# UMich-CURLY/SE3ET

Measured on AMD Instinct MI355X. Metric: point-cloud pairs/sec (fwd), SE3ET-E 5k-pt pairs, higher is better.
Workload: dtype f32

## Files before the change

### include/se3et_hip.h

```cpp
#ifndef SE3ET_HIP_H_
#define SE3ET_HIP_H_

#include <stddef.h>
#include <stdint.h>

#ifdef __cplusplus
extern "C" {
#endif

#define SE3_OK 0
#define SE3_ERR_INVALID_ARG 1
#define SE3_ERR_UNSUPPORTED 2
#define SE3_ERR_LAUNCH 3
#define SE3_ERR_WORKSPACE 4

#define SE3_MAX_BATCH 32
#define SE3_MAX_NEIGHBOR_LIMIT 64

const char* se3_version(void);
const char* se3_last_error(void);
void se3_debug_set_sinkhorn_variant(int variant);
unsigned long long se3_debug_dense_saturated_rows(int reset);
unsigned long long se3_debug_attention_saturated(int reset);
void se3_debug_kernel_timing(int enable);
int se3_debug_kernel_timing_collect_ex(float* microseconds, int* tags, double* aux, int capacity);

int se3_radius_neighbors(const float* q_points, int64_t nq, const float* s_points, int64_t ns,
                         const int64_t* q_lengths_host, const int64_t* s_lengths_host, int batch, float radius,
                         int limit, int64_t* neighbors, int32_t* max_count, void* stream);

int se3_neighbor_table_trim(const int64_t* full, int64_t rows, int full_width, int width, const int64_t* pair_row_ends_host,
                            const int* pair_widths_host, int num_pairs, int64_t* out, void* stream);
size_t se3_radius_grid_workspace_bytes(int64_t ns, int batch);
int se3_radius_grid_build(const float* s_points, int64_t ns, const int64_t* s_lengths_host, int batch, float radius,
                          void* workspace, size_t workspace_bytes, void* stream);
int se3_radius_neighbors_grid(const float* q_points, int64_t nq, const int64_t* q_lengths_host, const int64_t* s_lengths_host,
                              int64_t ns, int batch, const void* grid_workspace, float radius, int limit, int64_t* neighbors,
                              int32_t* max_count, int max_count_is_zero, void* stream);

int se3_radius_count_hist(const float* q_points, int64_t nq, const float* s_points, int64_t ns, const int64_t* q_lengths_host,
                          const int64_t* s_lengths_host, int batch, float radius, const void* grid_workspace, int hist_n,
                          const int* slot_of_cloud_host, int num_slots, int32_t* hist, int32_t* dropped, int32_t* max_count, void* stream);

int se3_radius_neighbors_ties(const float* q_points, int64_t nq, const float* s_points, int64_t ns, const int64_t* q_lengths_host,
                              const int64_t* s_lengths_host, int batch, float radius, int limit, int64_t* neighbors, int32_t* max_count,
                              int32_t* tie_rows, int32_t* tie_count, void* stream);
int se3_radius_neighbors_grid_ties(const float* q_points, int64_t nq, const int64_t* q_lengths_host, const int64_t* s_lengths_host,
                                   int64_t ns, int batch, const void* grid_workspace, float radius, int limit, int64_t* neighbors,
                                   int32_t* max_count, int max_count_is_zero, int32_t* tie_rows, int32_t* tie_count, void* stream);
size_t se3_kdtree_max_bytes(int64_t ns, int batch);
int se3_kdtree_build_host(const float* s_points_host, int64_t ns, const int64_t* s_lengths_host, int batch, void* tree_host, size_t capacity,
                          size_t* used_bytes);
size_t se3_radius_tie_scratch_bytes(int64_t num_tie_rows, int max_hits);
int se3_radius_neighbors_tie_order(const float* q_points, int64_t nq, const float* s_points, int64_t ns, const int64_t* q_lengths_host,
                                   const int64_t* s_lengths_host, int batch, const void* tree_dev, float radius, int limit,
                                   const int32_t* tie_rows, int64_t num_tie_rows, int max_hits, void* scratch, size_t scratch_bytes,
                                   int64_t* neighbors, void* stream);
int se3_debug_radius_tie_order_host(const float* q_points, int64_t nq, const float* s_points, int64_t ns, const int64_t* q_lengths,
                                    const int64_t* s_lengths, int batch, const void* tree_host, float radius, int limit,
                                    const int32_t* tie_rows, int64_t num_tie_rows, int max_hits, int64_t* neighbors, int* overflowed);
int64_t se3_debug_std_sort_host(const unsigned long long* keys, int64_t n, int mode);

size_t se3_grid_subsample_workspace_bytes(int64_t n, int batch);
int se3_grid_subsample(const float* points, const float* normals, int64_t n, const int64_t* lengths_host, int batch,
                       float voxel_size, float* s_points, float* s_normals, int64_t* s_lengths, void* workspace,
                       size_t workspace_bytes, void* stream);
int se3_grid_subsample_dev(const float* points, const float* normals, int64_t n_rows, const int64_t* lengths_dev, int batch,
                           float voxel_size, float* s_points, float* s_normals, int64_t* s_lengths, void* workspace,
                           size_t workspace_bytes, void* stream);

int se3_log_sinkhorn_fwd(const float* scores, const uint8_t* row_masks, const uint8_t* col_masks, const float* alpha,
                         int batch, int rows, int cols, int iterations, float inf, float* out, void* stream);
int se3_log_sinkhorn_bwd(const float* scores, const uint8_t* row_masks, const uint8_t* col_masks, const float* alpha,
                         const float* grad_out, int batch, int rows, int cols, int iterations, float inf, float* grad_scores,
                         float* grad_alpha_partial, void* stream);

size_t se3_group_norm_workspace_bytes(int64_t rows, int channels, int groups);
int se3_group_norm_fwd(const float* x, const float* x_bias, const float* residual, const float* weight, const float* bias,
                       int64_t rows, int channels, int groups, float eps, int apply_leaky_relu, float slope, float* out,
                       void* workspace, size_t workspace_bytes, void* stream);

int se3_group_norm_segments_fwd(const float* x, const float* x_bias, const float* residual, const float* weight,
                                const float* bias, int64_t rows, int channels, int groups,
                                const int64_t* segment_row_offsets_host, int num_segments, float eps, int apply_leaky_relu,
                                float slope, float* out, void* workspace, size_t workspace_bytes, void* stream);
size_t se3_group_norm_bwd_workspace_bytes(int channels);
int se3_group_norm_segments_bwd(const float* x, const float* x_bias, const float* residual, const float* weight, const float* bias,
                                const float* grad_out, int64_t rows, int channels, int groups, const int64_t* segment_row_offsets_host,
                                int num_segments, float eps, int apply_leaky_relu, float slope, float* grad_x, float* grad_residual,
                                float* grad_params, void* workspace, size_t workspace_bytes, void* stream);

size_t se3_group_norm_stats_workspace_bytes(int channels);
int se3_group_norm_stats(const float* x, const float* in_affine, float in_slope, const float* x_bias, const float* weight, const float* bias,
                         int64_t rows, int channels, int groups, const int64_t* segment_row_offsets_host, int num_segments, float eps,
                         float* affine_out, void* workspace, size_t workspace_bytes, void* stream);
int se3_group_norm_apply(const float* x, const float* affine_a, float slope_a, const float* affine_b, float slope_b, const float* residual,
                         const float* residual_affine, float final_slope, int64_t rows, int channels,
                         const int64_t* segment_row_offsets_host, int num_segments, int blocked_layout, float* out, void* stream);
int se3_group_norm_apply_amax(const float* x, const float* affine_a, float slope_a, const float* affine_b, float slope_b, const float* residual,
                              const float* residual_affine, float final_slope, int64_t rows, int channels,
                              const int64_t* segment_row_offsets_host, int num_segments, int blocked_layout, float* out, float* amax_out,
                              void* stream);
size_t se3_dense_norm_workspace_bytes(int groups);
int se3_dense_norm_fwd(const float* x, int64_t rows, int in_features, const float* in_affine_a, float in_slope_a, const float* in_affine_b,
                       float in_slope_b, const void* weight_pieces, int out_features, const float* linear_bias, const float* norm_weight,
                       const float* norm_bias, int groups, float eps, const int64_t* segment_row_offsets_host, int num_segments, float* out,
                       float* affine_out, void* workspace, size_t workspace_bytes, void* stream);
int se3_dense_residual_fwd(const float* x, int64_t rows, int in_features, const float* in_affine_a, float in_slope_a, const float* in_affine_b,
                           float in_slope_b, const void* weight_pieces, const float* affine, const float* x2, int in_features2,
                           const void* weight_pieces2, const float* affine2, const float* residual, int out_features, float final_slope,
                           const int64_t* segment_row_offsets_host, int num_segments, float* out, void* stream);
int se3_linear_stream(const float* x, int64_t rows, int in_features, int64_t x_row_stride, const void* weight_pieces, const float* bias,
                      int out_features, int apply_relu, float* out, int64_t out_row_stride, void* stream);
int se3_linear_stream_transposed(const float* x, int64_t rows, int in_features, int64_t x_row_stride, const void* weight_pieces,
                                 const float* bias, int out_features, int block_rows, float* out_t, int64_t ld, void* stream);

int se3_add_layer_norm_fwd(const float* hidden, const float* hidden_bias, const float* residual, const float* weight,
                           const float* bias, int64_t rows, int64_t residual_rows, int channels, float eps, float* out,
                           void* stream);
int se3_add_layer_norm_bwd(const float* hidden, const float* hidden_bias, const float* residual, const float* weight,
                           const float* grad_out, int64_t rows, int64_t residual_rows, int channels, float eps, float* grad_hidden,
                           float* grad_params, void* stream);

size_t se3_linear_weight_pieces_bytes(int out_features, int in_features);
int se3_linear_split_weights_f16(const float* weight, int out_features, int in_features, void* pieces, void* stream);
int se3_linear_f16(const float* x, int64_t rows, int in_features, int64_t x_row_stride, const void* weight_pieces, const float* bias,
                   int out_features, int apply_relu, float* out, int64_t out_row_stride, void* stream);

int se3_gather_rows_padded(const float* x, const int64_t* idx, int64_t n, int64_t m, int64_t width, float* out,
                           void* stream);
int se3_neighbor_max_pool(const float* x, const int64_t* idx, int64_t n, int64_t m, int nn, int64_t width, float* out,
                          void* stream);
int se3_neighbor_max_pool_bwd(const float* x, const int64_t* idx, const float* dout, int64_t n, int64_t m, int nn, int64_t width,
                              float* dx, void* stream);
int se3_anchor_max(const float* x, int num_anchors, int64_t rows, int channels, int64_t anchor_stride, int64_t row_stride,
// ... 774 lines not shown
```

### se3et_amd/csrc/radius_ties.hip

```cpp
#define SE3_EXACT_FP 1
#include "common.h"
#include "kdtree_ref.h"
#include <string.h>
#include <memory>
#include <thread>

namespace {

struct KdCloud {
  int32_t node_base;
  int32_t perm_base;
  int32_t n_nodes, n_points;
  float lo[3], hi[3];
  int32_t pad[2];
};
struct KdNode {
  int32_t kid0, kid1;
  int32_t first, last;
  int32_t axis;
  float low_end, high_start;
  int32_t pad;
};
struct KdHeader {
  int32_t magic, batch;
  int64_t total_nodes, total_points;
  int64_t off_clouds, off_perm, off_nodes;
  int64_t pad[2];
};
constexpr int32_t kMagic = 0x6b645433;
static_assert(sizeof(KdCloud) == 48 && sizeof(KdNode) == 32 && sizeof(KdHeader) == 64, "flattened k-d tree layout");

struct Batch {
  int64_t q_start[SE3_MAX_BATCH], q_count[SE3_MAX_BATCH], s_start[SE3_MAX_BATCH], s_count[SE3_MAX_BATCH];
  int n;
};

struct Strip {
  unsigned long long* base;
  int64_t stride;
  __host__ __device__ __forceinline__ unsigned long long get(int k) const { return base[(int64_t)k * stride]; }
  __host__ __device__ __forceinline__ void set(int k, unsigned long long v) const { base[(int64_t)k * stride] = v; }
};
__host__ __device__ __forceinline__ bool less_d2(unsigned long long a, unsigned long long b) { return (unsigned)(a >> 32) < (unsigned)(b >> 32); }

__host__ __device__ void adjust_heap(const Strip& s, int first, int hole, int len, unsigned long long value) {
  const int top = hole;
  int child = hole;
  while (child < (len - 1) / 2) {
    child = 2 * (child + 1);
    if (less_d2(s.get(first + child), s.get(first + child - 1))) child--;
    s.set(first + hole, s.get(first + child));
    hole = child;
  }
  if ((len & 1) == 0 && child == (len - 2) / 2) {
    child = 2 * (child + 1);
    s.set(first + hole, s.get(first + child - 1));
    hole = child - 1;
  }
  int parent = (hole - 1) / 2;
  while (hole > top && less_d2(s.get(first + parent), value)) {
    s.set(first + hole, s.get(first + parent));
    hole = parent;
    parent = (hole - 1) / 2;
  }
  s.set(first + hole, value);
}
__host__ __device__ void heap_sort(const Strip& s, int first, int last) {
  const int len = last - first;
  if (len >= 2) {
    for (int parent = (len - 2) / 2;; parent--) {
      adjust_heap(s, first, parent, len, s.get(first + parent));
      if (parent == 0) break;
    }
  }
  for (int end = last; end - first > 1;) {
    --end;
    const unsigned long long value = s.get(end);
    s.set(end, s.get(first));
    adjust_heap(s, first, 0, end - first, value);
  }
}
__host__ __device__ __forceinline__ void swap_at(const Strip& s, int a, int b) {
  const unsigned long long x = s.get(a), y = s.get(b);
  s.set(a, y);
  s.set(b, x);
}
__host__ __device__ __forceinline__ void linear_insert(const Strip& s, int last) {
  const unsigned long long val = s.get(last);
  int next = last - 1;
  while (less_d2(val, s.get(next))) {
    s.set(last, s.get(next));
    last = next;
    --next;
  }
  s.set(last, val);
}
__host__ __device__ void insertion_sort(const Strip& s, int first, int last) {
  if (first == last) return;
  for (int i = first + 1; i != last; ++i) {
    if (less_d2(s.get(i), s.get(first))) {
      const unsigned long long val = s.get(i);
      for (int k = i; k > first; k--) s.set(k, s.get(k - 1));
      s.set(first, val);
    } else {
      linear_insert(s, i);
    }
  }
}
struct Stacks {
  int* i;
  float* a;
  float* b;
  int stride;
};
constexpr int kMaxDepth = 48;

__host__ __device__ void std_sort(const Strip& s, int n, const Stacks& K) {
  if (n <= 0) return;
  constexpr int kThreshold = 16;
  int depth0 = 0;
  while ((2 << depth0) <= n) depth0++;
  int sp = 1;
  K.i[0] = 0 | (n << 16);
  K.a[0] = __builtin_bit_cast(float, 2 * depth0);
  while (sp > 0) {
    --sp;
    const int packed = K.i[sp * K.stride];
    int first = packed & 0xffff, last = (int)((unsigned)packed >> 16), depth = __builtin_bit_cast(int, K.a[sp * K.stride]);
    while (last - first > kThreshold) {
      if (depth == 0) {
        heap_sort(s, first, last);
        break;
      }
      --depth;
      const int mid = first + (last - first) / 2, a = first + 1, b = mid, c = last - 1;
      const unsigned long long va = s.get(a), vb = s.get(b), vc = s.get(c);
      int med;
      if (less_d2(va, vb)) med = less_d2(vb, vc) ? b : (less_d2(va, vc) ? c : a);
      else med = less_d2(va, vc) ? a : (less_d2(vb, vc) ? c : b);
      swap_at(s, first, med);
      const unsigned long long pivot = s.get(first);
      int lo = first + 1, hi = last;
      for (;;) {
        while (less_d2(s.get(lo), pivot)) ++lo;
        --hi;
        while (less_d2(pivot, s.get(hi))) --hi;
        if (!(lo < hi)) break;
        swap_at(s, lo, hi);
        ++lo;
      }
      if (sp < kMaxDepth) {
        K.i[sp * K.stride] = lo | (last << 16);
        K.a[sp * K.stride] = __builtin_bit_cast(float, depth);
        sp++;
      }
      last = lo;
    }
  }
  if (n > kThreshold) {
    insertion_sort(s, 0, kThreshold);
    for (int i = kThreshold; i < n; ++i) linear_insert(s, i);
  } else {
    insertion_sort(s, 0, n);
  }
}


__host__ __device__ bool tie_row(const float* __restrict__ q, const float* __restrict__ s, const Batch& bt, const unsigned char* __restrict__ tree,
                                 float r2, int limit, int64_t row, int max_hits, const Strip& strip, const Stacks& K, int64_t ns_total,
                                 int64_t* __restrict__ out) {
  int b = 0;
  while (b + 1 < bt.n && row >= bt.q_start[b] + bt.q_count[b]) b++;
  const KdHeader* H = reinterpret_cast<const KdHeader*>(tree);
  const KdCloud cl = reinterpret_cast<const KdCloud*>(tree + H->off_clouds)[b];
  const int32_t* perm = reinterpret_cast<const int32_t*>(tree + H->off_perm) + cl.perm_base;
  const KdNode* nodes = reinterpret_cast<const KdNode*>(tree + H->off_nodes) + cl.node_base;
  const float* sp = s + 3 * bt.s_start[b];
  const float qv[3] = {q[3 * row], q[3 * row + 1], q[3 * row + 2]};
  int n = 0;
  bool over = false;
  if (cl.n_points > 0) {
    float side[3] = {0.f, 0.f, 0.f}, outside = 0.f;
    for (int d = 0; d < 3; d++) {
      if (qv[d] < cl.lo[d]) { side[d] = (qv[d] - cl.lo[d]) * (qv[d] - cl.lo[d]); outside += side[d]; }
      if (qv[d] > cl.hi[d]) { side[d] = (qv[d] - cl.hi[d]) * (qv[d] - cl.hi[d]); outside += side[d]; }
    }
    int sp_ = 1;
    K.i[0] = 0;
    K.a[0] = outside;
    while (sp_ > 0) {
      const int top = (sp_ - 1) * K.stride;
      const int word = K.i[top], node = word & 0x3fffffff, stage = (int)((unsigned)word >> 30);
      const float f_outside = K.a[top];
      const KdNode nd = nodes[node];
      if (nd.kid0 < 0) {
        for (int k = nd.first; k < nd.last; k++) {
          const int j = perm[k];
          const float dx = qv[0] - sp[3 * j], dy = qv[1] - sp[3 * j + 1], dz = qv[2] - sp[3 * j + 2];
          float d2 = dx * dx;
          d2 += dy * dy;
          d2 += dz * dz;
          if (d2 < r2) {
            if (n < max_hits) strip.set(n, ((unsigned long long)__builtin_bit_cast(unsigned, d2) << 32) | (unsigned)(bt.s_start[b] + j));
            else over = true;
            n += n < max_hits ? 1 : 0;
          }
        }
        sp_--;
        continue;
      }
      const float v = nd.axis == 0 ? qv[0] : (nd.axis == 1 ? qv[1] : qv[2]);
      const float to_low = v - nd.low_end, to_high = v - nd.high_start;
      const bool low_first = (to_low + to_high) < 0;
      const float gap = low_first ? to_high * to_high : to_low * to_low;
      if (stage == 0) {
        K.i[top] = node | (1 << 30);
        if (sp_ < kMaxDepth) { K.i[sp_ * K.stride] = low_first ? nd.kid0 : nd.kid1; K.a[sp_ * K.stride] = f_outside; sp_++; } else { over = true; sp_--; }
      } else if (stage == 1) {
        const float kept = nd.axis == 0 ? side[0] : (nd.axis == 1 ? side[1] : side[2]);
        const float far_outside = f_outside + gap - kept;
        if (far_outside * 1.0f <= r2) {
          K.b[top] = kept;
          K.i[top] = node | (2 << 30);
          if (nd.axis == 0) side[0] = gap; else if (nd.axis == 1) side[1] = gap; else side[2] = gap;
          if (sp_ < kMaxDepth) { K.i[sp_ * K.stride] = low_first ? nd.kid1 : nd.kid0; K.a[sp_ * K.stride] = far_outside; sp_++; } else { over = true; sp_--; }
        } else {
          sp_--;
        }
      } else {
        const float kept = K.b[top];
        if (nd.axis == 0) side[0] = kept; else if (nd.axis == 1) side[1] = kept; else side[2] = kept;
        sp_--;
      }
    }
  }
  if (n >= 65536) over = true;
  if (over) return false;
  std_sort(strip, n, K);
  for (int k = 0; k < limit; k++) out[row * limit + k] = k < n ? (int64_t)(unsigned)(strip.get(k) & 0xffffffffull) : ns_total;
  return true;
}

__global__ __launch_bounds__(64) void radius_tie_rows_kernel(const float* __restrict__ q, const float* __restrict__ s, Batch bt,
                                                             const unsigned char* __restrict__ tree, float r2, int limit,
                                                             const int32_t* __restrict__ rows, int64_t num_rows, int max_hits,
                                                             unsigned long long* __restrict__ scratch, int64_t ns_total,
                                                             int64_t* __restrict__ out, int32_t* __restrict__ overflow) {
  __shared__ int stk_i[kMaxDepth * 64];
  __shared__ float stk_a[kMaxDepth * 64], stk_b[kMaxDepth * 64];
  const int64_t r = (int64_t)blockIdx.x * blockDim.x + threadIdx.x;
  if (r >= num_rows) return;
  const Stacks K{stk_i + threadIdx.x, stk_a + threadIdx.x, stk_b + threadIdx.x, 64};
  if (!tie_row(q, s, bt, tree, r2, limit, rows[r], max_hits, Strip{scratch + r, num_rows}, K, ns_total, out)) atomicAdd(overflow, 1);
}

int fill_batch(Batch* bt, const int64_t* q_len, const int64_t* s_len, int batch, int64_t nq, int64_t ns) {
  int64_t qs = 0, ss = 0;
  bt->n = batch;
  for (int b = 0; b < batch; b++) {
    if (q_len[b] < 0 || s_len[b] < 0) return 1;
    bt->q_start[b] = qs; bt->q_count[b] = q_len[b];
    bt->s_start[b] = ss; bt->s_count[b] = s_len[b];
    qs += q_len[b]; ss += s_len[b];
  }
  return qs != nq || ss != ns;
}

}

extern "C" size_t se3_kdtree_max_bytes(int64_t ns, int batch) {
  if (ns < 0 || batch < 1 || batch > SE3_MAX_BATCH) return 0;
  return se3_align256(sizeof(KdHeader)) + se3_align256(sizeof(KdCloud) * (size_t)batch) + se3_align256(sizeof(int32_t) * (size_t)(ns + 1)) +
         se3_align256(sizeof(KdNode) * (size_t)(2 * ns + batch));
}

extern "C" int se3_kdtree_build_host(const float* s_points_host, int64_t ns, const int64_t* s_lengths_host, int batch, void* tree_host,
                                     size_t capacity, size_t* used_bytes) {
  SE3_REQUIRE(s_points_host && s_lengths_host && tree_host && used_bytes, SE3_ERR_INVALID_ARG, "kdtree_build_host: null pointer");
  SE3_REQUIRE(batch >= 1 && batch <= SE3_MAX_BATCH && ns >= 0 && ns < (1ll << 30), SE3_ERR_INVALID_ARG, "kdtree_build_host: bad batch / size");
  SE3_REQUIRE(capacity >= se3_kdtree_max_bytes(ns, batch), SE3_ERR_WORKSPACE, "kdtree_build_host: buffer too small");
  unsigned char* base = (unsigned char*)tree_host;
  KdHeader H{};
  H.magic = kMagic;
  H.batch = batch;
  H.off_clouds = (int64_t)se3_align256(sizeof(KdHeader));
  H.off_perm = H.off_clouds + (int64_t)se3_align256(sizeof(KdCloud) * (size_t)batch);
  H.off_nodes = H.off_perm + (int64_t)se3_align256(sizeof(int32_t) * (size_t)(ns + 1));
  KdCloud* clouds = (KdCloud*)(base + H.off_clouds);
  int32_t* perm = (int32_t*)(base + H.off_perm);
  KdNode* nodes = (KdNode*)(base + H.off_nodes);
  std::vector<int64_t> start((size_t)batch + 1, 0);
  for (int b = 0; b < batch; b++) {
    SE3_REQUIRE(s_lengths_host[b] >= 0 && start[(size_t)b] + s_lengths_host[b] <= ns, SE3_ERR_INVALID_ARG, "kdtree_build_host: lengths exceed the point count");
    start[(size_t)b + 1] = start[(size_t)b] + s_lengths_host[b];
  }
  std::vector<std::unique_ptr<se3_kd::KdTree>> trees((size_t)batch);
  auto build_one = [&](int b) {
    const int64_t n = s_lengths_host[b];
    if (n > 0) trees[(size_t)b].reset(new se3_kd::KdTree(s_points_host + 3 * start[(size_t)b], n));
  };
  if (batch > 1 && ns >= 4096) {
    for (int b0 = 0; b0 < batch; b0 += 16) {
      std::vector<std::thread> pool;
      for (int b = b0; b < batch && b < b0 + 16; b++) pool.emplace_back(build_one, b);
      for (auto& t : pool) t.join();
    }
  } else {
    for (int b = 0; b < batch; b++) build_one(b);
  }
  int64_t s0 = 0, n0 = 0;
  for (int b = 0; b < batch; b++) {
    const int64_t n = s_lengths_host[b];
    KdCloud c{};
    c.node_base = (int32_t)n0;
    c.perm_base = (int32_t)s0;
    c.n_points = (int32_t)n;
    if (n > 0) {
      const se3_kd::KdTree& tree = *trees[(size_t)b];
      const auto& tn = tree.nodes();
      const auto& tp = tree.perm();
      c.n_nodes = (int32_t)tn.size();
      for (int d = 0; d < 3; d++) { c.lo[d] = tree.box_lo()[d]; c.hi[d] = tree.box_hi()[d]; }
      for (size_t k = 0; k < tp.size(); k++) perm[s0 + (int64_t)k] = (int32_t)tp[k];
      for (size_t k = 0; k < tn.size(); k++) {
        KdNode o{};
        o.kid0 = tn[k].kid[0]; o.kid1 = tn[k].kid[1];
        o.first = (int32_t)tn[k].first; o.last = (int32_t)tn[k].last;
        o.axis = tn[k].axis; o.low_end = tn[k].low_end; o.high_start = tn[k].high_start;
        nodes[n0 + (int64_t)k] = o;
      }
    }
    clouds[b] = c;
    s0 += n;
    n0 += c.n_nodes;
  }
  SE3_REQUIRE(s0 == ns, SE3_ERR_INVALID_ARG, "kdtree_build_host: lengths do not sum to ns");
  H.total_nodes = n0;
  H.total_points = ns;
  memcpy(base, &H, sizeof(H));
  *used_bytes = (size_t)H.off_nodes + sizeof(KdNode) * (size_t)n0;
  return SE3_OK;
}

extern "C" size_t se3_radius_tie_scratch_bytes(int64_t num_rows, int max_hits) {
  if (num_rows < 0 || max_hits < 0) return 0;
  return se3_align256(sizeof(unsigned long long) * (size_t)num_rows * (size_t)(max_hits > 0 ? max_hits : 1)) + 256;
}

extern "C" int se3_radius_neighbors_tie_order(const float* q_points, int64_t nq, const float* s_points, int64_t ns, const int64_t* q_lengths_host,
                                              const int64_t* s_lengths_host, int batch, const void* tree_dev, float radius, int limit,
                                              const int32_t* tie_rows, int64_t num_tie_rows, int max_hits, void* scratch, size_t scratch_bytes,
                                              int64_t* neighbors, void* stream) {
  SE3_REQUIRE(q_points && s_points && q_lengths_host && s_lengths_host && tree_dev && tie_rows && scratch && neighbors, SE3_ERR_INVALID_ARG,
              "radius_neighbors_tie_order: null pointer");
  SE3_REQUIRE(batch >= 1 && batch <= SE3_MAX_BATCH && limit >= 1 && limit <= SE3_MAX_NEIGHBOR_LIMIT && max_hits >= 1, SE3_ERR_INVALID_ARG,
              "radius_neighbors_tie_order: bad batch / limit / max_hits");
  SE3_REQUIRE(scratch_bytes >= se3_radius_tie_scratch_bytes(num_tie_rows, max_hits), SE3_ERR_WORKSPACE, "radius_neighbors_tie_order: scratch too small");
  Batch bt;
  SE3_REQUIRE(fill_batch(&bt, q_lengths_host, s_lengths_host, batch, nq, ns) == 0, SE3_ERR_INVALID_ARG,
              "radius_neighbors_tie_order: lengths do not sum to the sizes");
  if (num_tie_rows <= 0) return SE3_OK;
  hipStream_t st = (hipStream_t)stream;
  int32_t* overflow = (int32_t*)((char*)scratch + se3_radius_tie_scratch_bytes(num_tie_rows, max_hits) - 256);
  if (hipMemsetAsync(overflow, 0, sizeof(int32_t), st) != hipSuccess) {
    se3_set_error("radius_neighbors_tie_order: memset failed");
    return SE3_ERR_LAUNCH;
  }
  radius_tie_rows_kernel<<<(unsigned)se3_cdiv(num_tie_rows, 64), 64, 0, st>>>(q_points, s_points, bt, (const unsigned char*)tree_dev, radius * radius, limit,
                                                                               tie_rows, num_tie_rows, max_hits, (unsigned long long*)scratch, ns,
                                                                               neighbors, overflow);
  SE3_CHECK_LAUNCH("radius_neighbors_tie_order");
  return SE3_OK;
}

extern "C" int se3_debug_radius_tie_order_host(const float* q_points, int64_t nq, const float* s_points, int64_t ns, const int64_t* q_lengths,
                                               const int64_t* s_lengths, int batch, const void* tree_host, float radius, int limit,
                                               const int32_t* tie_rows, int64_t num_tie_rows, int max_hits, int64_t* neighbors, int* overflowed) {
  SE3_REQUIRE(q_points && s_points && q_lengths && s_lengths && tree_host && neighbors && overflowed && (tie_rows || num_tie_rows == 0),
              SE3_ERR_INVALID_ARG, "debug_radius_tie_order_host: null pointer");
  SE3_REQUIRE(batch >= 1 && batch <= SE3_MAX_BATCH && limit >= 1 && max_hits >= 1, SE3_ERR_INVALID_ARG, "debug_radius_tie_order_host: bad arguments");
  Batch bt;
  SE3_REQUIRE(fill_batch(&bt, q_lengths, s_lengths, batch, nq, ns) == 0, SE3_ERR_INVALID_ARG, "debug_radius_tie_order_host: lengths do not sum to the sizes");
  std::vector<unsigned long long> strip((size_t)max_hits);
  int si[kMaxDepth];
  float sa[kMaxDepth], sb[kMaxDepth];
  const Stacks K{si, sa, sb, 1};
  *overflowed = 0;
  for (int64_t r = 0; r < num_tie_rows; r++)
    if (!tie_row(q_points, s_points, bt, (const unsigned char*)tree_host, radius * radius, limit, tie_rows[r], max_hits, Strip{strip.data(), 1}, K, ns, neighbors))
      *overflowed += 1;
  return SE3_OK;
}

extern "C" int64_t se3_debug_std_sort_host(const unsigned long long* keys, int64_t n, int mode) {
  if (keys == nullptr || n < 0 || n >= 65536) return -1;
  std::vector<unsigned long long> a(keys, keys + n), b(keys, keys + n);
  auto cmp = [](unsigned long long x, unsigned long long y) { return (unsigned)(x >> 32) < (unsigned)(y >> 32); };
  const Strip strip{a.data(), 1};
  int si[kMaxDepth];
  float sa[kMaxDepth], sb[kMaxDepth];
  if (mode == 0) {
    std_sort(strip, (int)n, Stacks{si, sa, sb, 1});
    std::sort(b.begin(), b.end(), cmp);
  } else {
    heap_sort(strip, 0, (int)n);
    std::partial_sort(b.begin(), b.end(), b.end(), cmp);
  }
  int64_t diff = 0;
  for (int64_t i = 0; i < n; i++) diff += a[(size_t)i] != b[(size_t)i];
  return diff;
}
```

### se3et_amd/ops.py

```python
import ctypes
import os
import threading

import torch

from .caches import CACHE_EPOCH, Derived, Workspace, _Shared, also_clear, clear_caches, clear_weight_caches, validate_weight_caches
from ._lib import CONSTANTS, ENUMS, check, lib
from .stacking import PAIR_MAX_PAIRS, device_offsets, exclusive_offsets, to_device


_HAS_BLAS_SWITCH = hasattr(torch.backends.cuda, 'preferred_blas_library')
if _HAS_BLAS_SWITCH:
    torch.backends.cuda.preferred_blas_library('cublas')
_BLAS_SWITCH_LOCK = threading.Lock()
_BIG_GEMM_FLOP = 2.0e9


def mm(a, b):
    big = 2.0 * a.shape[0] * a.shape[1] * b.shape[1] > _BIG_GEMM_FLOP
    if _HAS_BLAS_SWITCH and big and (b.stride(-1) == 1 or a.shape[1] <= 32):
        with _BLAS_SWITCH_LOCK:
            torch.backends.cuda.preferred_blas_library('cublaslt')
            try:
                return torch.mm(a, b)
# ... 191 lines not shown
            max_count = _req(zeroed_max_count, torch.int32, 'zeroed_max_count', 1)
            if max_count.shape[0] != nb or not max_count.is_contiguous():
                raise RuntimeError('radius search: zeroed_max_count must be a contiguous (batch,) int32 tensor')
        else:
            max_count = torch.empty((nb,), dtype=torch.int32, device=q_points.device)
        tr, tc = _tie_buffers(ties, nq)
        check(lib().se3_radius_neighbors_grid_ties(q_points.data_ptr(), nq, ql, self.lengths, self.ns, self.batch, self.ws.data_ptr(),
                                                   self.radius, int(limit), out.data_ptr(), max_count.data_ptr(),
                                                   1 if zeroed_max_count is not None else 0, tr, tc, _stream()),
              'se3_radius_neighbors_grid')
        return out, max_count


def _tie_buffers(ties, nq):
    if ties is None:
        return None, None
    rows, count = ties
    _req(rows, torch.int32, 'tie_rows', 1), _req(count, torch.int32, 'tie_count', 1)
    if rows.shape[0] < nq or count.shape[0] != 1:
        raise RuntimeError('radius search: tie_rows needs room for every query row, tie_count is ONE int32 word')
    return rows.data_ptr(), count.data_ptr()


def radius_neighbors(q_points, s_points, q_lengths, s_lengths, radius, limit, grid=None, zeroed_max_count=None, ties=None):
    _req(q_points, torch.float32, 'q_points', 2)
    _req(s_points, torch.float32, 's_points', 2)
    if grid is None and s_points.shape[0] >= GRID_SEARCH_MIN_SUPPORT:
        grid = RadiusGrid(s_points, s_lengths, radius)
    if grid is not None:
        if grid.s_points.data_ptr() != s_points.data_ptr() or grid.radius != float(radius):
            raise RuntimeError('radius_neighbors: the grid was built for another support cloud / radius')
        return grid.search(q_points, q_lengths, limit, zeroed_max_count, ties)
    ql, nb = _host_lengths(q_lengths, 'q_lengths')
    sl, nb2 = _host_lengths(s_lengths, 's_lengths')
    if nb != nb2:
        raise RuntimeError('q_lengths and s_lengths differ in batch size')
    nq, ns = q_points.shape[0], s_points.shape[0]
    out = torch.empty((nq, limit), dtype=torch.int64, device=q_points.device)
    max_count = torch.empty((nb,), dtype=torch.int32, device=q_points.device)
    tr, tc = _tie_buffers(ties, nq)
    check(lib().se3_radius_neighbors_ties(q_points.data_ptr(), nq, s_points.data_ptr(), ns, ql, sl, nb, float(radius),
                                          int(limit), out.data_ptr(), max_count.data_ptr(), tr, tc, _stream()),
          'se3_radius_neighbors')
    return out, max_count


def radius_count_hist(q_points, s_points, q_lengths, s_lengths, radius, hist_n, slots, hist=None, grid=None, dropped=None, max_count=None):
    _req(q_points, torch.float32, 'q_points', 2)
    _req(s_points, torch.float32, 's_points', 2)
    ql, nb = _host_lengths(q_lengths, 'q_lengths')
    sl, nb2 = _host_lengths(s_lengths, 's_lengths')
    slots = [int(v) for v in (slots.tolist() if torch.is_tensor(slots) else slots)]
    if nb != nb2 or nb != len(slots):
        raise RuntimeError('radius_count_hist: q_lengths, s_lengths and slots differ in batch size')
    hist_n = int(hist_n)
    if hist is None:
        if not 1 <= hist_n <= 4096 or not slots or min(slots) < 0:
            raise RuntimeError('radius_count_hist: hist_n %d not in [1,4096], or no / negative slots' % hist_n)
        hist = torch.zeros((max(slots) + 1, hist_n), dtype=torch.int32, device=q_points.device)
    _req(hist, torch.int32, 'hist', 2)
    num_slots = hist.shape[0]
    if hist.shape[1] != hist_n:
        raise RuntimeError('radius_count_hist: hist must be (num_slots, hist_n)')
    dropped = torch.zeros((num_slots,), dtype=torch.int32, device=q_points.device) if dropped is None else _req(dropped, torch.int32, 'dropped', 1)
    max_count = torch.zeros((nb,), dtype=torch.int32, device=q_points.device) if max_count is None else _req(max_count, torch.int32, 'max_count', 1)
    if dropped.shape[0] != num_slots or max_count.shape[0] != nb:
        raise RuntimeError('radius_count_hist: dropped must be (num_slots,), max_count (batch,)')
    if grid is None and s_points.shape[0] >= GRID_SEARCH_MIN_SUPPORT:
        grid = RadiusGrid(s_points, s_lengths, radius)
    ws = None
    if grid is not None and grid is not False:
        if grid.s_points.data_ptr() != s_points.data_ptr() or grid.radius != float(radius) or grid.batch != nb:
            raise RuntimeError('radius_count_hist: the grid was built for another support cloud / radius')
        ws = grid.ws.data_ptr()
    check(lib().se3_radius_count_hist(q_points.data_ptr(), q_points.shape[0], s_points.data_ptr(), s_points.shape[0], ql, sl, nb, float(radius),
                                      ws, hist_n, (ctypes.c_int * nb)(*slots), num_slots, hist.data_ptr(), dropped.data_ptr(),
                                      max_count.data_ptr(), _stream()), 'se3_radius_count_hist')
    return hist, dropped, max_count


RADIUS_REFERENCE_TIES = os.environ.get('SE3_RADIUS_REFERENCE_TIES', '1') != '0'


class ReferenceTree:

    def __init__(self, s_points, s_lengths):
        self.s_points = _req(s_points, torch.float32, 's_points', 2)
        self.lengths, self.batch = _host_lengths(s_lengths, 's_lengths')
        self.ns = s_points.shape[0]
        host_pts = s_points.cpu()
        cap = lib().se3_kdtree_max_bytes(self.ns, self.batch)
        host = torch.empty((cap,), dtype=torch.uint8)
        used = ctypes.c_size_t(0)
        check(lib().se3_kdtree_build_host(host_pts.data_ptr(), self.ns, self.lengths, self.batch, host.data_ptr(), cap, ctypes.byref(used)),
              'se3_kdtree_build_host')
        self.tree = host[:int(used.value)].to(s_points.device)


def radius_tie_order(neighbors, q_points, s_points, q_lengths, s_lengths, radius, tie_rows, num_tie_rows, max_hits, tree=None):
    if num_tie_rows <= 0:
        return tree
    _req(neighbors, torch.int64, 'neighbors', 2)
    tree = tree if tree is not None else ReferenceTree(s_points, s_lengths)
    if tree.s_points.data_ptr() != s_points.data_ptr():
        raise RuntimeError('radius_tie_order: the tree was built for another support cloud')
    ql, nb = _host_lengths(q_lengths, 'q_lengths')
    nbytes = lib().se3_radius_tie_scratch_bytes(int(num_tie_rows), int(max_hits))
    scratch = torch.empty((nbytes,), dtype=torch.uint8, device=q_points.device)
    check(lib().se3_radius_neighbors_tie_order(q_points.data_ptr(), q_points.shape[0], s_points.data_ptr(), s_points.shape[0], ql, tree.lengths,
                                               nb, tree.tree.data_ptr(), float(radius), neighbors.shape[1], tie_rows.data_ptr(),
                                               int(num_tie_rows), int(max_hits), scratch.data_ptr(), nbytes, neighbors.data_ptr(), _stream()),
          'se3_radius_neighbors_tie_order')
    if not hasattr(_tie_tls, 'words'):
        _tie_tls.words = []
    _tie_tls.words.append(scratch[nbytes - 256:nbytes - 252].view(torch.int32))
    return tree


_tie_tls = threading.local()


def tie_overflow_check():
    words = getattr(_tie_tls, 'words', None)
    if not words:
        return
    _tie_tls.words = []
    left = int(torch.cat(words).sum())
    if left:
        raise RuntimeError('radius search: %d row(s) with exactly tied distances could not be given the reference order (more matches than the '
                           'search counted, or a k-d tree deeper than %d levels)' % (left, 48))


def radius_search_reference_order(q_points, s_points, q_lengths, s_lengths, radius, limit):
    nq = q_points.shape[0]
    flags = torch.zeros((nq + 1,), dtype=torch.int32, device=q_points.device) if RADIUS_REFERENCE_TIES else None
    ties = (flags[1:], flags[:1]) if flags is not None else None
    full, max_count = radius_neighbors(q_points, s_points, q_lengths, s_lengths, radius, limit, ties=ties)
    host = torch.cat((max_count.max().reshape(1), flags[:1])).tolist() if flags is not None else [int(max_count.max()), 0]
    if host[1] > 0:
        radius_tie_order(full, q_points, s_points, q_lengths, s_lengths, radius, flags[1:], host[1], max(host[0], 1))
        tie_overflow_check()
    return full, host[0]


def grid_subsample(points, lengths, normals, voxel_size):
    _req(points, torch.float32, 'points', 2)
    if normals is not None:
        _req(normals, torch.float32, 'normals', 2)
    if torch.is_tensor(lengths) and lengths.is_cuda:
        ld = _req(lengths.contiguous(), torch.int64, 'lengths', 1)
        n, nb, dev = points.shape[0], ld.shape[0], points.device
        ws_bytes = lib().se3_grid_subsample_workspace_bytes(n, nb)
        ws = torch.empty((ws_bytes,), dtype=torch.uint8, device=dev)
        s_points = torch.empty((n, 3), dtype=torch.float32, device=dev)
        s_normals = torch.empty((n, 3), dtype=torch.float32, device=dev) if normals is not None else None
        s_lengths = torch.empty((nb,), dtype=torch.int64, device=dev)
        check(lib().se3_grid_subsample_dev(points.data_ptr(), normals.data_ptr() if normals is not None else None, n, ld.data_ptr(), nb,
                                           float(voxel_size), s_points.data_ptr(), s_normals.data_ptr() if s_normals is not None else None,
                                           s_lengths.data_ptr(), ws.data_ptr(), ws_bytes, _stream()), 'se3_grid_subsample_dev')
        return s_points, s_normals, s_lengths
    ln, nb = _host_lengths(lengths, 'lengths')
    n = points.shape[0]
    dev = points.device
    ws_bytes = lib().se3_grid_subsample_workspace_bytes(n, nb)
    ws = torch.empty((ws_bytes,), dtype=torch.uint8, device=dev)
    s_points = torch.empty((n, 3), dtype=torch.float32, device=dev)
    s_normals = torch.empty((n, 3), dtype=torch.float32, device=dev) if normals is not None else None
    s_lengths = torch.empty((nb,), dtype=torch.int64, device=dev)
    check(lib().se3_grid_subsample(points.data_ptr(), normals.data_ptr() if normals is not None else None, n, ln, nb,
                                   float(voxel_size), s_points.data_ptr(),
                                   s_normals.data_ptr() if s_normals is not None else None, s_lengths.data_ptr(),
                                   ws.data_ptr(), ws_bytes, _stream()), 'se3_grid_subsample')
    return s_points, s_normals, s_lengths

# ... 2804 lines not shown
```

Baseline: 461.6.

## Build tie-order k-d tree on device and process tie rows per wavefront

Adds a GPU k-d tree build kernel: one block per cloud builds levels breadth-first, with the cloud held in LDS when it fits. This replaces the host build, which copied points to the CPU and the tree back to the device. The tie-order kernel now gives each row a whole wavefront, using ballot-based compaction of leaf hits into an LDS strip and falling back to global scratch when the strip overflows. The device build must reproduce the host tree's split choices exactly to keep the neighbour order, and the per-wave row layout sorts serially on lane 0.

```diff
diff --git a/include/se3et_hip.h b/include/se3et_hip.h
--- a/include/se3et_hip.h
+++ b/include/se3et_hip.h
@@ -51,6 +51,11 @@
 size_t se3_kdtree_max_bytes(int64_t ns, int batch);
 int se3_kdtree_build_host(const float* s_points_host, int64_t ns, const int64_t* s_lengths_host, int batch, void* tree_host, size_t capacity,
                           size_t* used_bytes);
+size_t se3_kdtree_build_workspace_bytes(int64_t ns, int batch);
+int se3_kdtree_build_device(const float* s_points, int64_t ns, const int64_t* s_lengths_host, int batch, void* tree_dev, size_t capacity,
+                            void* workspace, size_t workspace_bytes, void* stream);
+int se3_debug_kdtree_build_levels_host(const float* s_points_host, int64_t ns, const int64_t* s_lengths_host, int batch, void* tree_host,
+                                       size_t capacity, size_t* used_bytes);
 size_t se3_radius_tie_scratch_bytes(int64_t num_tie_rows, int max_hits);
 int se3_radius_neighbors_tie_order(const float* q_points, int64_t nq, const float* s_points, int64_t ns, const int64_t* q_lengths_host,
                                    const int64_t* s_lengths_host, int batch, const void* tree_dev, float radius, int limit,
diff --git a/se3et_amd/csrc/kdtree_build_core.h b/se3et_amd/csrc/kdtree_build_core.h
--- /dev/null
+++ b/se3et_amd/csrc/kdtree_build_core.h
@@ -0,0 +1,167 @@
+#pragma once
+#include <stdint.h>
+
+#if defined(__HIPCC__)
+#define SE3_KD_HD __host__ __device__ __forceinline__
+#else
+#define SE3_KD_HD inline
+#endif
+
+namespace se3_kdb {
+
+struct KdCloud {
+  int32_t node_base;
+  int32_t perm_base;
+  int32_t n_nodes, n_points;
+  float lo[3], hi[3];
+  int32_t pad[2];
+};
+struct KdNode {
+  int32_t kid0, kid1;
+  int32_t first, last;
+  int32_t axis;
+  float low_end, high_start;
+  int32_t pad;
+};
+struct KdHeader {
+  int32_t magic, batch;
+  int64_t total_nodes, total_points;
+  int64_t off_clouds, off_perm, off_nodes;
+  int64_t pad[2];
+};
+constexpr int32_t kMagic = 0x6b645433;
+constexpr int kLeafSize = 10;
+static_assert(sizeof(KdCloud) == 48 && sizeof(KdNode) == 32 && sizeof(KdHeader) == 64, "flattened k-d tree layout");
+
+struct OneLane {
+  static constexpr int width = 1;
+  int lane() const { return 0; }
+  float min(float v) const { return v; }
+  float max(float v) const { return v; }
+  int sum(int v) const { return v; }
+  int rank(bool flag, int* total) const { *total = flag ? 1 : 0; return 0; }
+  void sync() const {}
+  int take2(int* counter) const { const int v = *counter; *counter = v + 2; return v; }
+};
+
+struct Cloud {
+  const float* p;
+  int32_t* perm;
+  int32_t* tmp;
+  KdNode* nodes;
+  float* boxes;
+};
+
+template <class Lanes>
+SE3_KD_HD void tight_box(const Lanes& L, const Cloud& c, int first, int last, float (&mn)[3], float (&mx)[3]) {
+  const int j0 = c.perm[first];
+  for (int d = 0; d < 3; d++) mn[d] = mx[d] = c.p[3 * j0 + d];
+  for (int k = first + L.lane(); k < last; k += Lanes::width) {
+    const int j = c.perm[k];
+    for (int d = 0; d < 3; d++) {
+      const float v = c.p[3 * j + d];
+      if (v < mn[d]) mn[d] = v;
+      if (v > mx[d]) mx[d] = v;
+    }
+  }
+  for (int d = 0; d < 3; d++) { mn[d] = L.min(mn[d]); mx[d] = L.max(mx[d]); }
+}
+
+template <class Lanes>
+SE3_KD_HD void exchange_sweep(const Lanes& L, const Cloud& c, int first, int count, int axis, float cut, bool strict, int from, int boundary) {
+  int n_left = 0, n_right = 0;
+  for (int k0 = from; k0 < count; k0 += Lanes::width) {
+    const int k = k0 + L.lane();
+    bool left = false, right = false;
+    if (k < count) {
+      const float v = c.p[3 * c.perm[first + k] + axis];
+      const bool has = strict ? v < cut : v <= cut;
+      left = k < boundary && !has;
+      right = k >= boundary && has;
+    }
+    int tl, tr;
+    const int rl = L.rank(left, &tl), rr = L.rank(right, &tr);
+    if (left) c.tmp[first + n_left + rl] = k;
+    if (right) c.tmp[first + count - 1 - (n_right + rr)] = k;
+    n_left += tl;
+    n_right += tr;
+  }
+  L.sync();
+  for (int i = L.lane(); i < n_left; i += Lanes::width) {
+    const int a = first + c.tmp[first + i], b = first + c.tmp[first + count - n_left + i];
+    const int32_t x = c.perm[a];
+    c.perm[a] = c.perm[b];
+    c.perm[b] = x;
+  }
+  L.sync();
+}
+
+template <class Lanes>
+SE3_KD_HD void cut_node(const Lanes& L, const Cloud& c, int me, int* next_node) {
+  const int first = c.nodes[me].first, last = c.nodes[me].last, count = last - first;
+  float lo[3], hi[3], mn[3], mx[3];
+  for (int d = 0; d < 3; d++) { lo[d] = c.boxes[6 * me + d]; hi[d] = c.boxes[6 * me + 3 + d]; }
+  tight_box(L, c, first, last, mn, mx);
+  const float eps = 0.00001f;
+  float widest = hi[0] - lo[0];
+  for (int d = 1; d < 3; d++) widest = widest < hi[d] - lo[d] ? hi[d] - lo[d] : widest;
+  int axis = 0;
+  float best_spread = -1.f;
+  for (int d = 0; d < 3; d++)
+    if (hi[d] - lo[d] > (1 - eps) * widest) {
+      if (mx[d] - mn[d] > best_spread) { axis = d; best_spread = mx[d] - mn[d]; }
+    }
+  const float amn = axis == 0 ? mn[0] : (axis == 1 ? mn[1] : mn[2]), amx = axis == 0 ? mx[0] : (axis == 1 ? mx[1] : mx[2]);
+  const float alo = axis == 0 ? lo[0] : (axis == 1 ? lo[1] : lo[2]), ahi = axis == 0 ? hi[0] : (axis == 1 ? hi[1] : hi[2]);
+  const float mid = (alo + ahi) / 2;
+  const float cut = mid < amn ? amn : (mid > amx ? amx : mid);
+  int below = 0, upto = 0;
+  for (int k = first + L.lane(); k < last; k += Lanes::width) {
+    const float v = c.p[3 * c.perm[k] + axis];
+    below += v < cut ? 1 : 0;
+    upto += v <= cut ? 1 : 0;
+  }
+  below = L.sum(below);
+  upto = L.sum(upto);
+  exchange_sweep(L, c, first, count, axis, cut, true, 0, below);
+  exchange_sweep(L, c, first, count, axis, cut, false, below, upto);
+  const int half = count / 2;
+  int split = below > half ? below : (upto < half ? upto : half);
+  split = split < 1 ? 1 : (split > count - 1 ? count - 1 : split);
+  float low_end = c.p[3 * c.perm[first] + axis], high_start = c.p[3 * c.perm[first + split] + axis];
+  for (int k = first + L.lane(); k < last; k += Lanes::width) {
+    const float v = c.p[3 * c.perm[k] + axis];
+    if (k < first + split) low_end = v > low_end ? v : low_end;
+    else high_start = v < high_start ? v : high_start;
+  }
+  low_end = L.max(low_end);
+  high_start = L.min(high_start);
+  const int kid = L.take2(next_node);
+  if (L.lane() == 0) {
+    KdNode nd = c.nodes[me];
+    nd.kid0 = kid;
+    nd.kid1 = kid + 1;
+    nd.axis = axis;
+    nd.low_end = low_end;
+    nd.high_start = high_start;
+    c.nodes[me] = nd;
+    for (int s = 0; s < 2; s++) {
+      c.nodes[kid + s] = KdNode{-1, -1, s == 0 ? first : first + split, s == 0 ? first + split : last, 0, 0.f, 0.f, 0};
+      for (int d = 0; d < 3; d++) {
+        c.boxes[6 * (kid + s) + d] = (s == 1 && d == axis) ? cut : lo[d];
+        c.boxes[6 * (kid + s) + 3 + d] = (s == 0 && d == axis) ? cut : hi[d];
+      }
+    }
+  }
+}
+
+template <class Lanes>
+SE3_KD_HD void open_root(const Lanes& L, const Cloud& c, int n, float (&mn)[3], float (&mx)[3]) {
+  tight_box(L, c, 0, n, mn, mx);
+  if (L.lane() == 0) {
+    c.nodes[0] = KdNode{-1, -1, 0, n, 0, 0.f, 0.f, 0};
+    for (int d = 0; d < 3; d++) { c.boxes[d] = mn[d]; c.boxes[3 + d] = mx[d]; }
+  }
+}
+
+}
diff --git a/se3et_amd/csrc/radius_ties.hip b/se3et_amd/csrc/radius_ties.hip
--- a/se3et_amd/csrc/radius_ties.hip
+++ b/se3et_amd/csrc/radius_ties.hip
@@ -1,34 +1,17 @@
 #define SE3_EXACT_FP 1
 #include "common.h"
 #include "kdtree_ref.h"
+#include "kdtree_build_core.h"
 #include <string.h>
 #include <memory>
 #include <thread>
 
 namespace {
 
-struct KdCloud {
-  int32_t node_base;
-  int32_t perm_base;
-  int32_t n_nodes, n_points;
-  float lo[3], hi[3];
-  int32_t pad[2];
-};
-struct KdNode {
-  int32_t kid0, kid1;
-  int32_t first, last;
-  int32_t axis;
-  float low_end, high_start;
-  int32_t pad;
-};
-struct KdHeader {
-  int32_t magic, batch;
-  int64_t total_nodes, total_points;
-  int64_t off_clouds, off_perm, off_nodes;
-  int64_t pad[2];
-};
-constexpr int32_t kMagic = 0x6b645433;
-static_assert(sizeof(KdCloud) == 48 && sizeof(KdNode) == 32 && sizeof(KdHeader) == 64, "flattened k-d tree layout");
+using se3_kdb::KdCloud;
+using se3_kdb::KdHeader;
+using se3_kdb::KdNode;
+using se3_kdb::kMagic;
 
 struct Batch {
   int64_t q_start[SE3_MAX_BATCH], q_count[SE3_MAX_BATCH], s_start[SE3_MAX_BATCH], s_count[SE3_MAX_BATCH];
@@ -166,9 +149,40 @@
 }
 
 
-__host__ __device__ bool tie_row(const float* __restrict__ q, const float* __restrict__ s, const Batch& bt, const unsigned char* __restrict__ tree,
-                                 float r2, int limit, int64_t row, int max_hits, const Strip& strip, const Stacks& K, int64_t ns_total,
-                                 int64_t* __restrict__ out) {
+struct WaveLanes {
+  static constexpr int width = SE3_WAVE;
+  __device__ __forceinline__ int lane() const { return se3_lane(); }
+  __device__ __forceinline__ float min(float v) const {
+#pragma unroll
+    for (int o = 32; o > 0; o >>= 1) { const float w = __shfl_xor(v, o); v = w < v ? w : v; }
+    return v;
+  }
+  __device__ __forceinline__ float max(float v) const {
+#pragma unroll
+    for (int o = 32; o > 0; o >>= 1) { const float w = __shfl_xor(v, o); v = w > v ? w : v; }
+    return v;
+  }
+  __device__ __forceinline__ int sum(int v) const { return se3_wave_sum(v); }
+  __device__ __forceinline__ int rank(bool flag, int* total) const {
+    const unsigned long long m = __ballot(flag);
+    *total = __popcll(m);
+    return __popcll(m & ((1ull << se3_lane()) - 1ull));
+  }
+  __device__ __forceinline__ void sync() const {
+    __threadfence_block();
+    __builtin_amdgcn_wave_barrier();
+  }
+  __device__ __forceinline__ int take2(int* counter) const {
+    int v = 0;
+    if (se3_lane() == 0) v = atomicAdd(counter, 2);
+    return __shfl(v, 0);
+  }
+};
+
+template <class Lanes>
+__host__ __device__ bool tie_row(const Lanes& L, const float* __restrict__ q, const float* __restrict__ s, const Batch& bt,
+                                 const unsigned char* __restrict__ tree, float r2, int limit, int64_t row, int max_hits, const Strip& strip,
+                                 const Stacks& K, int64_t ns_total, int64_t* __restrict__ out) {
   int b = 0;
   while (b + 1 < bt.n && row >= bt.q_start[b] + bt.q_count[b]) b++;
   const KdHeader* H = reinterpret_cast<const KdHeader*>(tree);
@@ -194,17 +208,24 @@
       const float f_outside = K.a[top];
       const KdNode nd = nodes[node];
       if (nd.kid0 < 0) {
-        for (int k = nd.first; k < nd.last; k++) {
-          const int j = perm[k];
-          const float dx = qv[0] - sp[3 * j], dy = qv[1] - sp[3 * j + 1], dz = qv[2] - sp[3 * j + 2];
-          float d2 = dx * dx;
-          d2 += dy * dy;
-          d2 += dz * dz;
-          if (d2 < r2) {
-            if (n < max_hits) strip.set(n, ((unsigned long long)__builtin_bit_cast(unsigned, d2) << 32) | (unsigned)(bt.s_start[b] + j));
-            else over = true;
-            n += n < max_hits ? 1 : 0;
+        for (int k0 = nd.first; k0 < nd.last; k0 += Lanes::width) {
+          const int k = k0 + L.lane();
+          bool hit = false;
+          unsigned long long key = 0;
+          if (k < nd.last) {
+            const int j = perm[k];
+            const float dx = qv[0] - sp[3 * j], dy = qv[1] - sp[3 * j + 1], dz = qv[2] - sp[3 * j + 2];
+            float d2 = dx * dx;
+            d2 += dy * dy;
+            d2 += dz * dz;
+            hit = d2 < r2;
+            key = ((unsigned long long)__builtin_bit_cast(unsigned, d2) << 32) | (unsigned)(bt.s_start[b] + j);
           }
+          int hits;
+          const int at = n + L.rank(hit, &hits);
+          if (hit && at < max_hits) strip.set(at, key);
+          over = over || n + hits > max_hits;
+          n = n + hits < max_hits ? n + hits : max_hits;
         }
         sp_--;
         continue;
@@ -236,22 +257,32 @@
   }
   if (n >= 65536) over = true;
   if (over) return false;
-  std_sort(strip, n, K);
-  for (int k = 0; k < limit; k++) out[row * limit + k] = k < n ? (int64_t)(unsigned)(strip.get(k) & 0xffffffffull) : ns_total;
+  L.sync();
+  if (L.lane() == 0) std_sort(strip, n, K);
+  L.sync();
+  for (int k = L.lane(); k < limit; k += Lanes::width) out[row * limit + k] = k < n ? (int64_t)(unsigned)(strip.get(k) & 0xffffffffull) : ns_total;
   return true;
 }
 
-__global__ __launch_bounds__(64) void radius_tie_rows_kernel(const float* __restrict__ q, const float* __restrict__ s, Batch bt,
-                                                             const unsigned char* __restrict__ tree, float r2, int limit,
-                                                             const int32_t* __restrict__ rows, int64_t num_rows, int max_hits,
-                                                             unsigned long long* __restrict__ scratch, int64_t ns_total,
-                                                             int64_t* __restrict__ out, int32_t* __restrict__ overflow) {
-  __shared__ int stk_i[kMaxDepth * 64];
-  __shared__ float stk_a[kMaxDepth * 64], stk_b[kMaxDepth * 64];
-  const int64_t r = (int64_t)blockIdx.x * blockDim.x + threadIdx.x;
+constexpr int kTieWaves = 4;
+constexpr int kLdsStrip = 256;
+__global__ __launch_bounds__(kTieWaves * SE3_WAVE) void radius_tie_rows_kernel(const float* __restrict__ q, const float* __restrict__ s, Batch bt,
+                                                                                const unsigned char* __restrict__ tree, float r2, int limit,
+                                                                                const int32_t* __restrict__ rows, int64_t num_rows, int max_hits,
+                                                                                unsigned long long* __restrict__ scratch, int64_t ns_total,
+                                                                                int64_t* __restrict__ out, int32_t* __restrict__ overflow) {
+  __shared__ int stk_i[kTieWaves][kMaxDepth];
+  __shared__ float stk_a[kTieWaves][kMaxDepth], stk_b[kTieWaves][kMaxDepth];
+  __shared__ unsigned long long hits[kTieWaves][kLdsStrip];
+  const int wave = threadIdx.x / SE3_WAVE;
+  const int64_t r = (int64_t)blockIdx.x * kTieWaves + wave;
   if (r >= num_rows) return;
-  const Stacks K{stk_i + threadIdx.x, stk_a + threadIdx.x, stk_b + threadIdx.x, 64};
-  if (!tie_row(q, s, bt, tree, r2, limit, rows[r], max_hits, Strip{scratch + r, num_rows}, K, ns_total, out)) atomicAdd(overflow, 1);
+  const WaveLanes L;
+  const Stacks K{stk_i[wave], stk_a[wave], stk_b[wave], 1};
+  const int64_t row = rows[r];
+  bool done = tie_row(L, q, s, bt, tree, r2, limit, row, max_hits < kLdsStrip ? max_hits : kLdsStrip, Strip{hits[wave], 1}, K, ns_total, out);
+  if (!done && max_hits > kLdsStrip) done = tie_row(L, q, s, bt, tree, r2, limit, row, max_hits, Strip{scratch + r, num_rows}, K, ns_total, out);
+  if (!done && L.lane() == 0) atomicAdd(overflow, 1);
 }
 
 int fill_batch(Batch* bt, const int64_t* q_len, const int64_t* s_len, int batch, int64_t nq, int64_t ns) {
@@ -265,6 +296,93 @@
   }
   return qs != nq || ss != ns;
 }
+
+constexpr int kBuildThreads = 1024;
+constexpr int kLdsPoints = 8000;
+static_assert(20 * kLdsPoints + 256 <= 160 * 1024, "the LDS-resident cloud of the k-d tree build");
+
+__host__ __device__ __forceinline__ int64_t node_base_of(int64_t s_start, int b) { return 2 * s_start + b; }
+
+template <bool kLds>
+__global__ __launch_bounds__(kBuildThreads) void kdtree_build_kernel(const float* __restrict__ s, Batch bt, unsigned char* __restrict__ tree, KdHeader H,
+                                                                     int32_t* __restrict__ tmp_ws, float* __restrict__ boxes_ws) {
+  __shared__ float sh_p[kLds ? 3 * kLdsPoints : 1];
+  __shared__ int32_t sh_perm[kLds ? kLdsPoints : 1], sh_tmp[kLds ? kLdsPoints : 1];
+  __shared__ int next_node;
+  const int b = blockIdx.x, n = (int)bt.s_count[b], tid = threadIdx.x, wave = tid / SE3_WAVE;
+  const int64_t start = bt.s_start[b], node_base = node_base_of(start, b);
+  if (b == 0 && tid == 0) *reinterpret_cast<KdHeader*>(tree) = H;
+  KdCloud* cloud = reinterpret_cast<KdCloud*>(tree + H.off_clouds) + b;
+  int32_t* perm = reinterpret_cast<int32_t*>(tree + H.off_perm) + start;
+  KdCloud rec{};
+  rec.node_base = (int32_t)node_base;
+  rec.perm_base = (int32_t)start;
+  rec.n_points = n;
+  if (n == 0) {
+    if (tid == 0) *cloud = rec;
+    return;
+  }
+  se3_kdb::Cloud c;
+  c.nodes = reinterpret_cast<KdNode*>(tree + H.off_nodes) + node_base;
+  c.boxes = boxes_ws + 6 * node_base;
+  if (kLds) {
+    for (int k = tid; k < 3 * n; k += kBuildThreads) sh_p[k] = s[3 * start + k];
+    c.p = sh_p;
+    c.perm = sh_perm;
+    c.tmp = sh_tmp;
+  } else {
+    c.p = s + 3 * start;
+    c.perm = perm;
+    c.tmp = tmp_ws + start;
+  }
+  for (int k = tid; k < n; k += kBuildThreads) c.perm[k] = k;
+  if (tid == 0) next_node = 1;
+  __syncthreads();
+  const WaveLanes L;
+  if (wave == 0) {
+    float mn[3], mx[3];
+    se3_kdb::open_root(L, c, n, mn, mx);
+    for (int d = 0; d < 3; d++) { rec.lo[d] = mn[d]; rec.hi[d] = mx[d]; }
+  }
+  __syncthreads();
+  for (int begin = 0, end = 1; begin < end;) {
+    for (int node = begin + wave; node < end; node += kBuildThreads / SE3_WAVE)
+      if (c.nodes[node].last - c.nodes[node].first > se3_kdb::kLeafSize) se3_kdb::cut_node(L, c, node, &next_node);
+    __syncthreads();
+    begin = end;
+    end = next_node;
+    __syncthreads();
+  }
+  if (kLds)
+    for (int k = tid; k < n; k += kBuildThreads) perm[k] = sh_perm[k];
+  if (tid == 0) {
+    rec.n_nodes = next_node;
+    *cloud = rec;
+  }
+}
+
+KdHeader tree_layout(int64_t ns, int batch) {
+  KdHeader H{};
+  H.magic = kMagic;
+  H.batch = batch;
+  H.total_points = ns;
+  H.off_clouds = (int64_t)se3_align256(sizeof(KdHeader));
+  H.off_perm = H.off_clouds + (int64_t)se3_align256(sizeof(KdCloud) * (size_t)batch);
+  H.off_nodes = H.off_perm + (int64_t)se3_align256(sizeof(int32_t) * (size_t)(ns + 1));
+  return H;
+}
+
+struct BuildWorkspace {
+  int32_t* tmp;
+  float* boxes;
+  size_t bytes;
+  BuildWorkspace(void* base, int64_t ns, int batch) {
+    Se3Carver carve(base);
+    tmp = carve.take<int32_t>((size_t)ns + 1);
+    boxes = carve.take<float>(6 * (size_t)(2 * ns + batch));
+    bytes = carve.bytes();
+  }
+};
 
 }
 
@@ -342,6 +460,79 @@
   return SE3_OK;
 }
 
+extern "C" size_t se3_kdtree_build_workspace_bytes(int64_t ns, int batch) {
+  if (ns < 0 || batch < 1 || batch > SE3_MAX_BATCH) return 0;
+  return BuildWorkspace(nullptr, ns, batch).bytes;
+}
+
+extern "C" int se3_kdtree_build_device(const float* s_points, int64_t ns, const int64_t* s_lengths_host, int batch, void* tree_dev, size_t capacity,
+                                       void* workspace, size_t workspace_bytes, void* stream) {
+  SE3_REQUIRE(s_points && s_lengths_host && tree_dev && workspace, SE3_ERR_INVALID_ARG, "kdtree_build_device: null pointer");
+  SE3_REQUIRE(batch >= 1 && batch <= SE3_MAX_BATCH && ns >= 0 && ns < (1ll << 29), SE3_ERR_INVALID_ARG, "kdtree_build_device: bad batch / size");
+  SE3_REQUIRE(capacity >= se3_kdtree_max_bytes(ns, batch), SE3_ERR_WORKSPACE, "kdtree_build_device: buffer too small");
+  const BuildWorkspace ws(workspace, ns, batch);
+  SE3_REQUIRE(workspace_bytes >= ws.bytes, SE3_ERR_WORKSPACE, "kdtree_build_device: workspace too small");
+  Batch bt{};
+  SE3_REQUIRE(fill_batch(&bt, s_lengths_host, s_lengths_host, batch, ns, ns) == 0, SE3_ERR_INVALID_ARG, "kdtree_build_device: lengths do not sum to ns");
+  KdHeader H = tree_layout(ns, batch);
+  H.total_nodes = node_base_of(ns, batch);
+  int64_t longest = 0;
+  for (int b = 0; b < batch; b++) longest = std::max(longest, s_lengths_host[b]);
+  hipStream_t st = (hipStream_t)stream;
+  if (longest <= kLdsPoints)
+    kdtree_build_kernel<true><<<batch, kBuildThreads, 0, st>>>(s_points, bt, (unsigned char*)tree_dev, H, ws.tmp, ws.boxes);
+  else
+    kdtree_build_kernel<false><<<batch, kBuildThreads, 0, st>>>(s_points, bt, (unsigned char*)tree_dev, H, ws.tmp, ws.boxes);
+  SE3_CHECK_LAUNCH("kdtree_build_device");
+  return SE3_OK;
+}
+
+extern "C" int se3_debug_kdtree_build_levels_host(const float* s_points_host, int64_t ns, const int64_t* s_lengths_host, int batch, void* tree_host,
+                                                  size_t capacity, size_t* used_bytes) {
+  SE3_REQUIRE(s_points_host && s_lengths_host && tree_host && used_bytes, SE3_ERR_INVALID_ARG, "debug_kdtree_build_levels_host: null pointer");
+  SE3_REQUIRE(batch >= 1 && batch <= SE3_MAX_BATCH && ns >= 0 && ns < (1ll << 29), SE3_ERR_INVALID_ARG, "debug_kdtree_build_levels_host: bad batch / size");
+  SE3_REQUIRE(capacity >= se3_kdtree_max_bytes(ns, batch), SE3_ERR_WORKSPACE, "debug_kdtree_build_levels_host: buffer too small");
+  Batch bt{};
+  SE3_REQUIRE(fill_batch(&bt, s_lengths_host, s_lengths_host, batch, ns, ns) == 0, SE3_ERR_INVALID_ARG,
+              "debug_kdtree_build_levels_host: lengths do not sum to ns");
+  unsigned char* base = (unsigned char*)tree_host;
+  KdHeader H = tree_layout(ns, batch);
+  H.total_nodes = node_base_of(ns, batch);
+  memcpy(base, &H, sizeof(H));
+  std::vector<int32_t> tmp((size_t)ns + 1);
+  std::vector<float> boxes(6 * (size_t)H.total_nodes);
+  const se3_kdb::OneLane L;
+  for (int b = 0; b < batch; b++) {
+    const int n = (int)bt.s_count[b];
+    const int64_t start = bt.s_start[b], node_base = node_base_of(start, b);
+    KdCloud rec{};
+    rec.node_base = (int32_t)node_base;
+    rec.perm_base = (int32_t)start;
+    rec.n_points = n;
+    if (n > 0) {
+      se3_kdb::Cloud c;
+      c.p = s_points_host + 3 * start;
+      c.perm = (int32_t*)(base + H.off_perm) + start;
+      c.tmp = tmp.data() + start;
+      c.nodes = (KdNode*)(base + H.off_nodes) + node_base;
+      c.boxes = boxes.data() + 6 * node_base;
+      for (int k = 0; k < n; k++) c.perm[k] = k;
+      int next_node = 1;
+      se3_kdb::open_root(L, c, n, rec.lo, rec.hi);
+      for (int begin = 0, end = 1; begin < end;) {
+        for (int node = begin; node < end; node++)
+          if (c.nodes[node].last - c.nodes[node].first > se3_kdb::kLeafSize) se3_kdb::cut_node(L, c, node, &next_node);
+        begin = end;
+        end = next_node;
+      }
+      rec.n_nodes = next_node;
+    }
+    ((KdCloud*)(base + H.off_clouds))[b] = rec;
+  }
+  *used_bytes = (size_t)H.off_nodes + sizeof(KdNode) * (size_t)H.total_nodes;
+  return SE3_OK;
+}
+
 extern "C" size_t se3_radius_tie_scratch_bytes(int64_t num_rows, int max_hits) {
   if (num_rows < 0 || max_hits < 0) return 0;
   return se3_align256(sizeof(unsigned long long) * (size_t)num_rows * (size_t)(max_hits > 0 ? max_hits : 1)) + 256;
@@ -366,7 +557,7 @@
     se3_set_error("radius_neighbors_tie_order: memset failed");
     return SE3_ERR_LAUNCH;
   }
-  radius_tie_rows_kernel<<<(unsigned)se3_cdiv(num_tie_rows, 64), 64, 0, st>>>(q_points, s_points, bt, (const unsigned char*)tree_dev, radius * radius, limit,
+  radius_tie_rows_kernel<<<(unsigned)se3_cdiv(num_tie_rows, kTieWaves), kTieWaves * SE3_WAVE, 0, st>>>(q_points, s_points, bt, (const unsigned char*)tree_dev, radius * radius, limit,
                                                                                tie_rows, num_tie_rows, max_hits, (unsigned long long*)scratch, ns,
                                                                                neighbors, overflow);
   SE3_CHECK_LAUNCH("radius_neighbors_tie_order");
@@ -387,7 +578,7 @@
   const Stacks K{si, sa, sb, 1};
   *overflowed = 0;
   for (int64_t r = 0; r < num_tie_rows; r++)
-    if (!tie_row(q_points, s_points, bt, (const unsigned char*)tree_host, radius * radius, limit, tie_rows[r], max_hits, Strip{strip.data(), 1}, K, ns, neighbors))
+    if (!tie_row(se3_kdb::OneLane{}, q_points, s_points, bt, (const unsigned char*)tree_host, radius * radius, limit, tie_rows[r], max_hits, Strip{strip.data(), 1}, K, ns, neighbors))
       *overflowed += 1;
   return SE3_OK;
 }
diff --git a/se3et_amd/ops.py b/se3et_amd/ops.py
--- a/se3et_amd/ops.py
+++ b/se3et_amd/ops.py
@@ -297,14 +297,26 @@
 RADIUS_REFERENCE_TIES = os.environ.get('SE3_RADIUS_REFERENCE_TIES', '1') != '0'
 
 
+TIE_TREE_ON_HOST = os.environ.get('SE3_TIE_TREE', 'device') == 'host'
+
+
 class ReferenceTree:
+    host_builds = 0
 
     def __init__(self, s_points, s_lengths):
         self.s_points = _req(s_points, torch.float32, 's_points', 2)
         self.lengths, self.batch = _host_lengths(s_lengths, 's_lengths')
         self.ns = s_points.shape[0]
+        cap = lib().se3_kdtree_max_bytes(self.ns, self.batch)
+        if not TIE_TREE_ON_HOST:
+            ws_bytes = lib().se3_kdtree_build_workspace_bytes(self.ns, self.batch)
+            self.tree = torch.empty((cap,), dtype=torch.uint8, device=s_points.device)
+            ws = torch.empty((ws_bytes,), dtype=torch.uint8, device=s_points.device)
+            check(lib().se3_kdtree_build_device(s_points.data_ptr(), self.ns, self.lengths, self.batch, self.tree.data_ptr(), cap, ws.data_ptr(),
+                                                ws_bytes, _stream()), 'se3_kdtree_build_device')
+            return
+        ReferenceTree.host_builds += 1
         host_pts = s_points.cpu()
-        cap = lib().se3_kdtree_max_bytes(self.ns, self.batch)
         host = torch.empty((cap,), dtype=torch.uint8)
         used = ctypes.c_size_t(0)
         check(lib().se3_kdtree_build_host(host_pts.data_ptr(), self.ns, self.lengths, self.batch, host.data_ptr(), cap, ctypes.byref(used)),
```

Result: no change. 465.9 (median of 6 runs) (+0.9%).
